# Bing-Jing/Ape-X

Measured on AMD Instinct MI355X. Metric: learner SGD steps/sec + actor frames/sec, Ape-X DQN Atari at 1/2/4/8 MI355X, higher is better.
Workload: dtype fp32

## Files before the change

### ape-x_amd/ops/csrc/f32_kernels.hip

```cpp
#include <algorithm>
#include <cstdio>
#include <cstdlib>
#include <type_traits>

#include "common.h"
#include "kernels.h"
#include "tree_dev.h"

namespace apex {
namespace {

typedef float f32x16 __attribute__((ext_vector_type(16)));
typedef float f32x4 __attribute__((ext_vector_type(4)));

__device__ __forceinline__ f32x4 ld4(const float* p) { return *reinterpret_cast<const f32x4*>(p); }
__device__ __forceinline__ f32x4 zero4() { return f32x4{0.f, 0.f, 0.f, 0.f}; }
__device__ __forceinline__ f32x4 u8x4(uint32_t w) {
  return f32x4{(float)(w & 0xFFu), (float)((w >> 8) & 0xFFu), (float)((w >> 16) & 0xFFu), (float)(w >> 24)};
}

constexpr int kPlane = 84 * 84;

typedef __amdgpu_buffer_rsrc_t Rsrc;
__device__ __forceinline__ Rsrc make_rsrc(const void* p, uint32_t nbytes) {
// ... 779 lines not shown
    return {(uint32_t)(((c.m0 + row) * 3136 + 4 * ch) * 4)};
  }
  static __device__ f32x4 load_a_row(const Args&, const Ctx& c, const RowA& r, int kb) {
    return bld4(c.in, r.off + (uint32_t)(kb * BK * 4));
  }
  static __device__ RowB row_b(const Args&, const Ctx& c, int nl, int ch) {
    return {(uint32_t)(((c.n0 + nl) * 3136 + 4 * ch) * 4)};
  }
  static __device__ f32x4 load_b_row(const Args&, const Ctx& c, const RowB& r, int kb) {
    return bld4(c.w, r.off + (uint32_t)(kb * BK * 4));
  }
};

constexpr int kPlaneDw = kPlane / 4;

struct W1Split {
  bfx8 hi[8], mid[8], lo[8];
};

__device__ __forceinline__ void split_w1(const float* wrow, W1Split& w) {
#pragma unroll
  for (int kb = 0; kb < 8; ++kb) {
    const f32x4 v0 = ld4(wrow + 32 * kb), v1 = ld4(wrow + 32 * kb + 8);
    const float x[8] = {v0[0], v0[1], v0[2], v0[3], v1[0], v1[1], v1[2], v1[3]};
    uint32_t h[4], m[4], l[4];
#pragma unroll
    for (int j = 0; j < 4; ++j) {
      const float a = x[2 * j], b = x[2 * j + 1];
      const float ah = trunc_bf16(a), bh = trunc_bf16(b);
      const float ar = a - ah, br = b - bh;
      const float am = trunc_bf16(ar), bm = trunc_bf16(br);
      h[j] = pack_bf16_hi(ah, bh);
      m[j] = pack_bf16_hi(am, bm);
      l[j] = pack_bf16_hi(ar - am, br - bm);
    }
    w.hi[kb] = __builtin_bit_cast(bfx8, make_uint4(h[0], h[1], h[2], h[3]));
    w.mid[kb] = __builtin_bit_cast(bfx8, make_uint4(m[0], m[1], m[2], m[3]));
    w.lo[kb] = __builtin_bit_cast(bfx8, make_uint4(l[0], l[1], l[2], l[3]));
  }
}

constexpr int kC1xGrid = 512;
constexpr int kC1xGridLearner = 384;
constexpr int kC1xDrawMax = 8;
constexpr int kC1xChunks = 4 * (kPlane / 16), kC1xPer = (kC1xChunks + 255) / 256;

__device__ __forceinline__ void c1x_load(const F32Set& set, int smp, uint4 (&v)[kC1xPer], const int* fid) {
  const int B = set.B, prob = smp / B, b = smp - prob * B, t = threadIdx.x;
  const F32Prob p = pick(set, prob);
  const uint8_t* fr = static_cast<const uint8_t*>(p.in);
  const FrameSrc f{fr, p.ids, p.idx};
  const uint4* s0 = reinterpret_cast<const uint4*>(fid ? fr + (size_t)fid[0] * kPlane : frame_plane(f, b, 0, kPlane));
  const uint4* s1 = reinterpret_cast<const uint4*>(fid ? fr + (size_t)fid[1] * kPlane : frame_plane(f, b, 1, kPlane));
  const uint4* s2 = reinterpret_cast<const uint4*>(fid ? fr + (size_t)fid[2] * kPlane : frame_plane(f, b, 2, kPlane));
  const uint4* s3 = reinterpret_cast<const uint4*>(fid ? fr + (size_t)fid[3] * kPlane : frame_plane(f, b, 3, kPlane));
#pragma unroll
  for (int k = 0; k < kC1xPer; ++k) {
    const int e = min(t + 256 * k, kC1xChunks - 1), c = e / 441;
    const uint4* sc = c == 0 ? s0 : (c == 1 ? s1 : (c == 2 ? s2 : s3));
    v[k] = sc[e - c * 441];
  }
}

__device__ __forceinline__ void c1x_store(const uint4 (&v)[kC1xPer], uint32_t* xs) {
  const int t = threadIdx.x;
#pragma unroll
  for (int k = 0; k < kC1xPer; ++k) {
    const int e = t + 256 * k;
    if (e < kC1xChunks) {
      const f32x4 a = u8x4(v[k].x), bq = u8x4(v[k].y), c = u8x4(v[k].z), d = u8x4(v[k].w);
      uint4* dst = reinterpret_cast<uint4*>(xs) + 2 * e;
      dst[0] = make_uint4(pack_bf16_hi(a[0], a[1]), pack_bf16_hi(a[2], a[3]), pack_bf16_hi(bq[0], bq[1]),
                          pack_bf16_hi(bq[2], bq[3]));
      dst[1] = make_uint4(pack_bf16_hi(c[0], c[1]), pack_bf16_hi(c[2], c[3]), pack_bf16_hi(d[0], d[1]),
                          pack_bf16_hi(d[2], d[3]));
    }
  }
}

__device__ __forceinline__ int opaque_i(int x) {
  asm volatile("" : "+v"(x));
  return x;
}
template <bool BITS>
__global__ __launch_bounds__(256, 2) void f32_conv1_fwd_x3_k(F32Set set, ConvSample cs) {
  __shared__ __attribute__((aligned(16))) uint32_t xs[2 * kPlaneDw * 4];
  __shared__ int fid[kC1xDrawMax][4];
  const int B = set.B, total = set.n * B;
  const int t = threadIdx.x, lane = t & 63, wave = t >> 6;
  const int i = lane & 15, q = lane >> 4, nh = wave >> 1;
  const bool draw = cs.out_idx != nullptr;
  const int G = draw ? cs.nhost : (int)gridDim.x;
  if (draw && (int)blockIdx.x >= G) {
    staged_scatter(cs.rows, blockIdx.x - G);
    return;
  }
  const __bf16* xb = reinterpret_cast<const __bf16*>(xs);
  W1Split w;
  int cur = -1;
  uint4 v[kC1xPer];
  const int per = (total + G - 1) / G;
  const int s0 = blockIdx.x * per, s1 = min(total, s0 + per);
  if (draw) {
    for (int k = wave; k < s1 - s0; k += 4) {
      const int smp = s0 + k, prob = smp / B, b = smp - prob * B;
      const int64_t len64 = cs.length[0];
      const int length = (int)(len64 < (int64_t)cs.t.size[0] ? len64 : (int64_t)cs.t.size[0]);
      const float pmin = cs.t.node_min[cs.t.levels - 1][0];
      float p;
      const int node = tree_sample_leaf(cs.t, b, B, length, cs.exclude_last, cs.seed, (uint64_t)cs.counter[0], lane,
                                        &p);
      const int se = staged_row_of(cs.rows, node, lane);
      const F32Prob pp = pick(set, prob);
      const int* ids = se < 0 ? pp.ids : (pp.ids == cs.rows.dst.s_ids ? cs.rows.st.s_ids : cs.rows.st.s2_ids);
      const int srow = se < 0 ? node : se;
      const bool crow = prob == 0 && cs.batch_fid != nullptr;
      uint32_t f = 0;
      if (lane < 4) {
        f = (uint32_t)ids[4 * srow + lane];
      } else if (crow && lane < 7) {
        const void* col = lane == 4 ? (const void*)(se < 0 ? cs.src_act : cs.rows.st.action)
                                    : (lane == 5 ? (const void*)(se < 0 ? cs.src_rew : cs.rows.st.reward)
                                                 : (const void*)(se < 0 ? cs.src_done : cs.rows.st.done));
        f = static_cast<const uint32_t*>(col)[srow];
      }
      if (lane < 4) fid[k][lane] = (int)f;
      if (prob == 0 && lane == 0) {
        cs.out_idx[b] = node;
        cs.out_w[b] = per_is_weight(p, pmin, 1.f, cs.beta[0]);
      }
      if (crow) {
        if (lane < 4) {
          cs.batch_fid[4 * b + lane] = (int)f;
        } else if (lane < 7) {
          void* dst = lane == 4 ? (void*)cs.batch_act : (lane == 5 ? (void*)cs.batch_rew : (void*)cs.batch_done);
          static_cast<uint32_t*>(dst)[b] = f;
        }
      }
    }
    __syncthreads();
  }
  if (s0 < s1) c1x_load(set, s0, v, draw ? fid[0] : nullptr);
  for (int smp = s0; smp < s1; ++smp) {
    const int prob = smp / B, b = smp - prob * B;
    const F32Prob p = pick(set, prob);
    if (prob != cur) {
      cur = prob;
      split_w1(p.w + (nh * 16 + i) * 256 + (q >> 1) * 16 + (q & 1) * 4, w);
    }
    __syncthreads();
    c1x_store(v, xs);
    __syncthreads();
    if (smp + 1 < s1) c1x_load(set, smp + 1, v, draw ? fid[smp + 1 - s0] : nullptr);
    float* out = p.out + (size_t)b * 400 * 32 + nh * 16 + 4 * q;
    uint16_t* bits =
        BITS && p.relu_bits ? reinterpret_cast<uint16_t*>(p.relu_bits + (size_t)b * 400) + nh : nullptr;
    float4 bias4;
    bias4.x = p.bias[nh * 16 + 4 * q];
    bias4.y = p.bias[nh * 16 + 4 * q + 1];
    bias4.z = p.bias[nh * 16 + 4 * q + 2];
    bias4.w = p.bias[nh * 16 + 4 * q + 3];
    auto frags = [&](int tile, bfx8 (&a)[8]) {
      const int m = tile * 16 + i, oy = m / 20, ox = m - oy * 20;
      const __bf16* a0 = xb + (4 * oy + 2 * (q >> 1)) * 84 + 4 * ox + 4 * (q & 1);
#pragma unroll
      for (int kb = 0; kb < 8; ++kb) {
        const uint2* ap = reinterpret_cast<const uint2*>(a0 + (kb >> 1) * kPlane + (kb & 1) * 4 * 84);
        const uint2 lo = ap[0], hi = ap[opaque_i(21)];
        a[kb] = __builtin_bit_cast(bfx8, make_uint4(lo.x, lo.y, hi.x, hi.y));
      }
    };
    auto tile_mfma = [&](int tile, const bfx8 (&a)[8], auto WB) {
      f32x4 ah = zero4(), am = zero4(), al = zero4();
#pragma unroll
      for (int kb = 0; kb < 8; ++kb) {
        ah = __builtin_amdgcn_mfma_f32_16x16x32_bf16(w.hi[kb], a[kb], ah, 0, 0, 0);
        am = __builtin_amdgcn_mfma_f32_16x16x32_bf16(w.mid[kb], a[kb], am, 0, 0, 0);
        al = __builtin_amdgcn_mfma_f32_16x16x32_bf16(w.lo[kb], a[kb], al, 0, 0, 0);
      }
      float4 y;
      y.x = fmaxf(ah[0] + (am[0] + al[0]) + bias4.x, 0.f);
      y.y = fmaxf(ah[1] + (am[1] + al[1]) + bias4.y, 0.f);
      y.z = fmaxf(ah[2] + (am[2] + al[2]) + bias4.z, 0.f);
      y.w = fmaxf(ah[3] + (am[3] + al[3]) + bias4.w, 0.f);
      *reinterpret_cast<float4*>(out + (size_t)(tile * 16 + i) * 32) = y;
      if constexpr (decltype(WB)::value) {
        const unsigned long long b0 = __ballot(y.x > 0.f), b1 = __ballot(y.y > 0.f), b2 = __ballot(y.z > 0.f),
                                 b3 = __ballot(y.w > 0.f);
        auto lo = [&](unsigned long long b) { return ((uint32_t)b >> i) & 0x00010001u; };
        auto hi = [&](unsigned long long b) { return ((uint32_t)(b >> 32) >> i) & 0x00010001u; };
        const uint32_t T = lo(b0) | lo(b1) << 1 | lo(b2) << 2 | lo(b3) << 3;
        const uint32_t U = hi(b0) | hi(b1) << 1 | hi(b2) << 2 | hi(b3) << 3;
        const uint32_t nb = (T & 0xFu) | ((T >> 12) & 0xF0u) | ((U & 0xFu) << 8) | ((U >> 4) & 0xF000u);
        bits[(tile * 16 + i) * 2] = (uint16_t)nb;
      }
    };
    auto tiles = [&](auto WB) {
      bfx8 fa[8], fb[8];
      const int t0 = wave & 1;
      frags(t0, fa);
      for (int pr = 0; pr < 6; ++pr) {
        const int tile = t0 + 4 * pr;
        frags(tile + 2, fb);
        tile_mfma(tile, fa, WB);
        frags(min(tile + 4, 24), fa);
        tile_mfma(tile + 2, fb, WB);
      }
      if (t0 == 0) tile_mfma(24, fa, WB);
    };
    if constexpr (BITS) {
      if (__builtin_amdgcn_readfirstlane(bits != nullptr)) tiles(std::true_type{});
      else tiles(std::false_type{});
    } else {
      tiles(std::false_type{});
    }
  }
}

struct BwdArgs {
  const void* x;
  const int* ids;
  const int* idx;
  const float* dy;
  const float* w;
  const float* mask;
  const uint32_t* mask_bits;
  const int* batch_fid;
  float* out;
  float* out2;
  int B;
  int kbps;
  int splits;
};

struct Fc1Dgrad {
  static constexpr int BM = 64, BN = 64, BK = 32, WM = 2;
  static constexpr bool A_KMAJ = true, B_KMAJ = false, SMEM = false;
  using Args = BwdArgs;
  using Smem = NoSmem;
  struct Ctx {
    int m0, n0, kb0, kb1;
    Rsrc dy, w;
  };
  static __host__ __device__ int tiles(int B) { return ((B + BM - 1) / BM) * 49; }
  static __device__ void decode(const Args& a, int block, Ctx& c, Smem&) {
    c.n0 = (block % 49) * BN;
    c.m0 = (block / 49) * BM;
    c.kb0 = 0;
    c.kb1 = 256 / BK;
    c.dy = make_rsrc(a.dy, (uint32_t)a.B * 256 * 4);
    c.w = make_rsrc(a.w, 256 * 3136 * 4);
  }
  using RowA = BufRow;
  using RowB = BufRow;
  static __device__ RowA row_a(const Args&, const Ctx& c, int row, int ch) {
    return {(uint32_t)((c.m0 + row) * 256 + 4 * ch) * 4};
  }
  static __device__ f32x4 load_a_row(const Args&, const Ctx& c, const RowA& r, int kb) {
    return bld4(c.dy, r.off + (uint32_t)(kb * BK * 4));
  }
  static __device__ RowB row_b(const Args&, const Ctx& c, int row, int ch) {
    return {(uint32_t)(row * 3136 + c.n0 + 4 * ch) * 4};
  }
  static __device__ f32x4 load_b_row(const Args&, const Ctx& c, const RowB& r, int kb) {
    return bld4(c.w, r.off + (uint32_t)(kb * BK * 3136 * 4));
  }
  static __device__ void store(const Args& a, const Ctx& c, int ml, int nl, float v) {
    const int b = c.m0 + ml;
    if (b >= a.B) return;
    const size_t o = (size_t)b * 3136 + c.n0 + nl;
    a.out[o] = a.mask[o] > 0.f ? v : 0.f;
  }
  static constexpr bool MASK_BITS = true;
  static __host__ __device__ bool use_bits(const Args& a) { return a.mask_bits != nullptr; }
  static __device__ uint32_t mask_word(const Args& a, const Ctx& c, int ml, int nl0) {
    return a.mask_bits[(size_t)min(c.m0 + ml, a.B - 1) * 98 + ((c.n0 + nl0) >> 5)];
  }
  static __device__ void store_keep(const Args& a, const Ctx& c, int ml, int nl, float v, bool keep) {
    const int b = c.m0 + ml;
    if (b < a.B) a.out[(size_t)b * 3136 + c.n0 + nl] = keep ? v : 0.f;
  }
};

struct Fc1Wgrad {
  static constexpr int BM = 64, BN = 64, BK = 32, WM = 2;
  static constexpr bool A_KMAJ = false, B_KMAJ = false, SMEM = false;
  using Args = BwdArgs;
  using Smem = NoSmem;
  struct Ctx {
// ... 362 lines not shown
  static __device__ RowB row_b(const Args&, const Ctx&, int n, int ch) { return {(uint32_t)(n * 64 + 4 * ch) * 4}; }
  static __device__ f32x4 load_b_row(const Args&, const Ctx& c, const RowB& r, int kb) {
    int ty, tx;
    tap_of(c, kb, ty, tx);
    const int ky = (c.cls >> 1) + 2 * ty, kx = (c.cls & 1) + 2 * tx;
    return bld4(c.w, r.off + (uint32_t)(((ky * 4 + kx) * 32 * 64 + (kb % KPT) * BK) * 4));
  }
  static __device__ void store(const Args& a, const Ctx& c, int ml, int n, float v) {
    const int b = c.b0 + ml;
    if (b >= a.B) return;
    const int iy = 2 * c.jy + (c.cls >> 1), ix = 2 * c.jx + (c.cls & 1);
    const size_t o = ((size_t)b * 400 + iy * 20 + ix) * 32 + n;
    a.out[o] = a.mask[o] > 0.f ? v : 0.f;
  }
  static constexpr bool MASK_BITS = true;
  static __host__ __device__ bool use_bits(const Args& a) { return a.mask_bits != nullptr; }
  static __device__ uint32_t mask_word(const Args& a, const Ctx& c, int ml, int) {
    const int iy = 2 * c.jy + (c.cls >> 1), ix = 2 * c.jx + (c.cls & 1);
    return a.mask_bits[(size_t)min(c.b0 + ml, a.B - 1) * 400 + iy * 20 + ix];
  }
  static __device__ void store_keep(const Args& a, const Ctx& c, int ml, int n, float v, bool keep) {
    const int b = c.b0 + ml;
    if (b >= a.B) return;
    const int iy = 2 * c.jy + (c.cls >> 1), ix = 2 * c.jx + (c.cls & 1);
    a.out[((size_t)b * 400 + iy * 20 + ix) * 32 + n] = keep ? v : 0.f;
  }
};
using Conv2DgradP = Conv2DgradPT<16>;
using Conv2DgradP32 = Conv2DgradPT<32>;

constexpr int kStageSplitDefault = 3 + 4 * 3 + 16 * (0 + 1);
constexpr int kBwdTileDefault = 1;

struct SplitPlan {
  int splits, kbps;
};

SplitPlan plan_splits(int kbt, int ntiles, int target_blocks) {
  int s = std::max(1, target_blocks / ntiles);
  int kbps = std::max(1, (kbt + s - 1) / s);
  s = (kbt + kbps - 1) / kbps;
  return {s, kbps};
}

SplitPlan wgrad_plan(int layer, int B, int target) {
  switch (layer) {
    case 1: {
      const int S = target == 1 ? 1 : kConv1WgradS;
      return {(B + S - 1) / S, S};
    }
    case 2: return plan_splits(ConvWgrad<2>::kblocks(B), 512 / 64, target > 0 ? target : 256);
    case 3: return plan_splits(ConvWgrad<3>::kblocks(B), 576 / 64, target > 0 ? target : 252);
    default: throw std::invalid_argument("f32 wgrad layer");
  }
}

int g_stage_split = -1;
int stage_split_mask() {
  if (g_stage_split < 0) {
    const char* e = std::getenv("APEX_F32_STAGE_SPLIT");
    g_stage_split = e ? std::atoi(e) : kStageSplitDefault;
  }
  return g_stage_split;
}

constexpr int kPrefetchDefault = 0;
int g_prefetch = -1;
int prefetch_mask() {
  if (g_prefetch < 0) {
    const char* e = std::getenv("APEX_F32_PREFETCH");
    g_prefetch = e ? std::atoi(e) : kPrefetchDefault;
  }
  return g_prefetch;
}
constexpr int kBatchResolveDefault = 1;
int g_batch_resolve = -1;
int batch_resolve_mask() {
  if (g_batch_resolve < 0) {
    const char* e = std::getenv("APEX_F32_BATCH_RESOLVE");
    g_batch_resolve = e ? std::atoi(e) & 3 : kBatchResolveDefault;
  }
  return g_batch_resolve;
}
int prefetch_depth(int cls) { return std::min(3, 1 + ((prefetch_mask() >> (2 * cls)) & 3)); }

template <class P, int D, bool XB>
void launch1_d(const typename P::Args& a, int blocks, hipStream_t s, int form) {
  switch (form) {
    case 1: gemm_k<P, 1, D, XB><<<blocks, 256, 0, s>>>(a); break;
    case 2: gemm_k<P, 2, D, XB><<<blocks, 256, 0, s>>>(a); break;
    case 3: gemm_k<P, 3, D, XB><<<blocks, 256, 0, s>>>(a); break;
    default: gemm_k<P, 0, D, XB><<<blocks, 256, 0, s>>>(a);
  }
}
template <class P, bool XB>
void launch1_x(const typename P::Args& a, int blocks, hipStream_t s, bool small) {
  const int m = stage_split_mask();
  const int form = small && ((m >> 4) & 3) ? ((m >> 4) & 3) - 1 : m & 3;
  switch (prefetch_depth(small ? 2 : 0)) {
    case 2: launch1_d<P, 2, XB>(a, blocks, s, form); break;
    case 3: launch1_d<P, 3, XB>(a, blocks, s, form); break;
    default: launch1_d<P, 1, XB>(a, blocks, s, form);
  }
}
template <class P>
void launch1(const typename P::Args& a, int blocks, hipStream_t s, bool small = false, bool bits = false) {
  if (blocks <= 0) return;
  if constexpr (HasReluBits<P>::value) {
    if (bits) launch1_x<P, true>(a, blocks, s, small);
    else launch1_x<P, false>(a, blocks, s, small);
  } else {
    launch1_x<P, false>(a, blocks, s, small);
  }
  LAUNCH_CHECK();
}

template <class P1, class P2, int D, bool XB>
void launch2_d(const typename P1::Args& a1, const typename P2::Args& a2, int n1, int nb, const TreeRide& r,
               hipStream_t s) {
  switch ((stage_split_mask() >> 2) & 3) {
    case 1: gemm2_k<P1, P2, 1, D, XB><<<nb, 256, 0, s>>>(a1, a2, n1, r); break;
    case 2: gemm2_k<P1, P2, 2, D, XB><<<nb, 256, 0, s>>>(a1, a2, n1, r); break;
    case 3: gemm2_k<P1, P2, 3, D, XB><<<nb, 256, 0, s>>>(a1, a2, n1, r); break;
    default: gemm2_k<P1, P2, 0, D, XB><<<nb, 256, 0, s>>>(a1, a2, n1, r);
  }
}
template <class P1, class P2, bool XB>
void launch2_x(const typename P1::Args& a1, const typename P2::Args& a2, int n1, int nb, const TreeRide& r,
               hipStream_t s) {
  switch (prefetch_depth(1)) {
    case 2: launch2_d<P1, P2, 2, XB>(a1, a2, n1, nb, r, s); break;
    case 3: launch2_d<P1, P2, 3, XB>(a1, a2, n1, nb, r, s); break;
    default: launch2_d<P1, P2, 1, XB>(a1, a2, n1, nb, r, s);
  }
}

template <class P1, class P2>
void launch2(const typename P1::Args& a1, int n1, const typename P2::Args& a2, int n2, hipStream_t s,
             const TreeRide* ride = nullptr) {
  if (n1 + n2 <= 0) return;
  TreeRide r{};
  if (ride && ride->stage) {
    r = *ride;
    r.nhost = n1 + n2;
  }
  const int nb = n1 + n2 + tree_ride_blocks(r);
  if (P2::use_bits(a2)) launch2_x<P1, P2, true>(a1, a2, n1, nb, r, s);
  else launch2_x<P1, P2, false>(a1, a2, n1, nb, r, s);
  LAUNCH_CHECK();
}

void check_set(const F32Set& set) {
  if (set.n < 1 || set.n > kMaxProbs) throw std::invalid_argument("f32: 1..3 problems");
  if (set.B <= 0) throw std::invalid_argument("f32: B must be positive");
  if ((int64_t)(set.B + 128) * 400 * 32 * 4 >= (int64_t)1 << 31)
    throw std::invalid_argument("f32: batch too large for 32-bit operand offsets");
}

template <class P>
void fwd_launch(const F32Set& set, hipStream_t s) {
  launch1<P>(set, set.n * P::tiles(set.B), s, set.n * set.B < 1024, set.p[0].relu_bits != nullptr);
}

}

void f32_set_stage_split(int mask) { g_stage_split = mask; }
int f32_stage_split() { return stage_split_mask(); }
void f32_set_prefetch(int mask) { g_prefetch = mask; }
int f32_prefetch() { return prefetch_mask(); }
void f32_set_batch_resolve(int mask) { g_batch_resolve = mask < 0 ? -1 : mask & 3; }
int f32_batch_resolve() { return batch_resolve_mask(); }

static bool learner_sized(const F32Set& set) { return set.n * set.B >= 1024; }

static int default_tile(int layer) {
  static int t2 = -1, t3 = -1;
  if (t2 < 0) {
    t2 = t3 = 0;
    if (const char* e = std::getenv("APEX_F32_TILES")) std::sscanf(e, "%d%*c%d", &t2, &t3);
  }
  return layer == 2 ? t2 : t3;
}

void f32_conv_fwd_multi(int layer, const F32Set& set, hipStream_t s, int c1_grid, int tile, const ConvSample* draw) {
  check_set(set);
  if (draw && draw->out_idx && layer != 1) throw std::invalid_argument("f32_conv_fwd_multi: the draw folds into conv1");
  if (tile == 0 && (layer == 2 || layer == 3)) tile = default_tile(layer);
  switch (layer) {
    case 1: {
      if (c1_grid <= 0) c1_grid = learner_sized(set) ? kC1xGridLearner : (set.n * set.B + 1) / 2;
      const int G = std::min(set.n * set.B, c1_grid > 0 ? c1_grid : kC1xGrid);
      ConvSample c{};
      if (draw && draw->out_idx) {
        c = *draw;
        c.nhost = G;
        if ((set.n * set.B + G - 1) / G > kC1xDrawMax)
          throw std::invalid_argument("f32 conv1 draw: <= 8 samples per workgroup");
        if (!c.length || !c.beta || !c.counter || !c.out_w || set.p[0].idx != c.out_idx)
          throw std::invalid_argument("f32 conv1 draw: fill level, beta, counter, weights, and problem 0 reading idx");
        if (c.batch_fid && (!c.batch_act || !c.batch_rew || !c.batch_done || !c.src_act || !c.src_rew || !c.src_done))
          throw std::invalid_argument("f32 conv1 draw: the compact rows need all four outputs and the table columns");
        for (int k = 0; k < set.n; ++k)
          if (!set.p[k].ids || (c.rows.E > 0 && set.p[k].ids != c.rows.dst.s_ids && set.p[k].ids != c.rows.dst.s2_ids))
            throw std::invalid_argument("f32 conv1 draw: every problem reads the replay's frame-id tables");
      }
      const int nb = G + (c.out_idx ? (c.rows.E + 255) / 256 : 0);
      if (set.p[0].relu_bits) f32_conv1_fwd_x3_k<true><<<nb, 256, 0, s>>>(set, c);
      else f32_conv1_fwd_x3_k<false><<<nb, 256, 0, s>>>(set, c);
      LAUNCH_CHECK();
      break;
    }
    case 2:
      if (learner_sized(set) && tile == 1) fwd_launch<Conv2FwdT<64, 64, 32, 2>>(set, s);
      else if (learner_sized(set) && tile == 2) fwd_launch<Conv2FwdT<128, 64, 32, 4>>(set, s);
      else if (learner_sized(set)) fwd_launch<Conv2FwdT<128, 64, 32, 2>>(set, s);
      else fwd_launch<Conv2FwdT<128, 32, 32, 4>>(set, s);
      break;
    case 3:
      if (learner_sized(set) && tile == 2) fwd_launch<Conv3FwdT<128, 64, 32, 2>>(set, s);
      else if (learner_sized(set) && tile == 3) fwd_launch<Conv3FwdT<128, 32, 32, 4>>(set, s);
      else if (learner_sized(set)) fwd_launch<Conv3FwdT<64, 64, 32, 2>>(set, s);
      else fwd_launch<Conv3FwdT<128, 64, 32, 2>>(set, s);
      break;
    default: throw std::invalid_argument("f32_conv_fwd_multi: layer must be 1, 2 or 3");
  }
}

int f32_fc1_splits() { return kFcSplits; }

int f32_fc1_fwd_multi(const F32Set& set, hipStream_t s) {
  check_set(set);
  fwd_launch<Fc1FwdT<64, 64, 32, 2>>(set, s);
  return kFcSplits;
}

constexpr int kFc1WgSlices = 1;

int f32_fc1_wgrad_splits() { return kFc1WgSlices; }

size_t f32_fc1_wgrad_workspace_floats() { return (size_t)kFc1WgSlices * 256 * 3136; }

static void check_bwd_batch(int B) {
  if ((int64_t)B * 400 * 32 * 4 + (int64_t)64 * 400 * 32 * 4 >= (int64_t)1 << 31)
    throw std::invalid_argument("f32 backward: batch too large for 32-bit operand offsets");
}

void f32_fc1_bwd_split(const float* dz, const float* a3, const float* wfc1p, float* dy3, float* ws, int B,
                       hipStream_t s, const TreeRide* ride, const uint32_t* mask_bits) {
  if (B <= 0) return;
  check_bwd_batch(B);
  BwdArgs d{};
  d.dy = dz;
  d.w = wfc1p;
  d.mask = a3;
  d.mask_bits = mask_bits;
  d.out = dy3;
  d.B = B;
  BwdArgs w{};
  w.x = a3;
  w.dy = dz;
  w.out = ws;
  w.B = B;
  const int nkb = (B + Fc1Wgrad::BK - 1) / Fc1Wgrad::BK;
  w.splits = std::min(kFc1WgSlices, nkb);
  w.kbps = (nkb + w.splits - 1) / w.splits;
  w.splits = (nkb + w.kbps - 1) / w.kbps;
  launch2<Fc1Wgrad, Fc1Dgrad>(w, Fc1Wgrad::tiles(B) * w.splits, d, Fc1Dgrad::tiles(B), s, ride);
}

int f32_fc1_wgrad_slices(int B) {
  const int nkb = (B + Fc1Wgrad::BK - 1) / Fc1Wgrad::BK;
  const int g = std::min(kFc1WgSlices, nkb), kbps = (nkb + g - 1) / g;
  return (nkb + kbps - 1) / kbps;
}

int f32_wgrad_splits(int layer, int B, int target) { return wgrad_plan(layer, B, target).splits; }

int f32_wgrad_kbps(int layer, int B, int target) { return wgrad_plan(layer, B, target).kbps; }

size_t f32_wgrad_workspace_floats(int layer, int B, int target) {
  const SplitPlan p = wgrad_plan(layer, B, target);
  const size_t per = layer == 1 ? 32 * 256 : (layer == 2 ? 64 * 512 : 64 * 576);
  const size_t cout = layer == 1 ? 32 : 64;
  return (size_t)p.splits * (per + cout);
}

void f32_conv_bwd(int layer, const void* x, const int* ids, const int* idx, const float* dy, const float* w,
                  const float* mask, float* dx, float* ws, int B, hipStream_t s, int target, int tile,
                  const TreeRide* ride, const uint32_t* mask_bits, const int* batch_fid) {
  if (B <= 0) return;
  check_bwd_batch(B);
// ... 95 lines not shown
```

### ape-x_amd/ops/csrc/hip_bindings.cpp

```cpp
#include <pybind11/pybind11.h>
#include <pybind11/stl.h>

#include <array>
#include <optional>
#include <vector>

#include "common.h"
#include "kernels.h"

namespace py = pybind11;
using namespace apex;

namespace {

template <typename T>
T* P(uint64_t v) {
  return reinterpret_cast<T*>(static_cast<uintptr_t>(v));
}
hipStream_t S(uint64_t v) { return reinterpret_cast<hipStream_t>(static_cast<uintptr_t>(v)); }

struct TreeHandle {
  TreeDesc d{};
};

// ... 431 lines not shown
        !a.delta || !a.lw || !(a.dz_bf || a.dz) || !a.part || !a.step)
      throw std::invalid_argument("dqn_heads_bwd: missing pointer");
    dqn_heads_bwd(a, S(s));
  });
  m.def("conv_wgrad", [](int layer, uint64_t x, uint64_t ids, uint64_t idx, uint64_t dy, uint64_t dy_mask, int B,
                         uint64_t ws, uint64_t grad, uint64_t bgrad, uint64_t s) {
    conv_wgrad(layer, P<const void>(x), P<const int>(ids), P<const int>(idx), P<const uint16_t>(dy),
               P<const uint16_t>(dy_mask), B, P<float>(ws), P<float>(grad), P<float>(bgrad), S(s));
  });
  m.def("pack_conv_wt", [](uint64_t src, uint64_t dst, int N, int C, int KH, int KW, uint64_t s) {
    pack_conv_wt(P<const float>(src), P<uint16_t>(dst), N, C, KH, KW, S(s));
  });
  auto f32set = [](const std::vector<std::vector<uint64_t>>& probs, int B) {
    if (probs.empty() || probs.size() > (size_t)kMaxProbs) throw std::invalid_argument("1..3 problems");
    F32Set set{};
    for (size_t i = 0; i < probs.size(); ++i) {
      const auto& t = probs[i];
      if (t.size() != 7 && t.size() != 8) throw std::invalid_argument("f32 problem: 7 or 8 fields");
      set.p[i] = F32Prob{P<const void>(t[0]), P<const int>(t[1]), P<const int>(t[2]), P<const float>(t[3]),
                         P<const float>(t[4]), P<const float>(t[5]), P<float>(t[6]),
                         t.size() == 8 ? P<uint32_t>(t[7]) : nullptr};
      if (set.p[i].relu_bits && i != 0) throw std::invalid_argument("f32 problem: sign bits are problem 0's");
    }
    set.n = (int)probs.size();
    set.B = B;
    return set;
  };
  m.def("f32_conv_fwd_multi", [f32set](int layer, const std::vector<std::vector<uint64_t>>& probs, int B,
                                       uint64_t s, int c1_grid, int tile, py::object draw) {
    f32_conv_fwd_multi(layer, f32set(probs, B), S(s), c1_grid, tile,
                       draw.is_none() ? nullptr : draw.cast<const ConvSample*>());
  }, py::arg("layer"), py::arg("probs"), py::arg("B"), py::arg("s"), py::arg("c1_grid") = 0, py::arg("tile") = 0,
     py::arg("draw") = py::none());
  py::class_<ConvSample>(m, "ConvSample");
  m.def("make_conv_sample", [](const TreeHandle& t, uint64_t length_ptr, uint64_t beta_ptr, uint64_t seed,
                               uint64_t counter, uint64_t out_idx, uint64_t out_w, int exclude_last,
                               py::object rows_stage, py::object rows_dst, uint64_t rows_slot, uint64_t rows_prio,
                               int rows_E, uint64_t batch_fid, uint64_t batch_act, uint64_t batch_rew,
                               uint64_t batch_done, py::object batch_src) {
    if (!length_ptr || !beta_ptr || !counter || !out_idx || !out_w)
      throw std::invalid_argument("make_conv_sample: fill level, beta, counter, idx and weight pointers");
    ConvSample c{};
    c.t = t.d;
    c.length = P<const int64_t>(length_ptr);
    c.beta = P<const float>(beta_ptr);
    c.counter = P<const int64_t>(counter);
    c.seed = seed;
    c.out_idx = P<int>(out_idx);
    c.out_w = P<float>(out_w);
    c.exclude_last = exclude_last;
    if (rows_E > 0) {
      if (!rows_slot || !rows_prio) throw std::invalid_argument("make_conv_sample: staged slots / priorities");
      c.rows = StagedRows{trans_table(rows_stage.cast<py::dict>()), trans_table(rows_dst.cast<py::dict>()),
                          P<const int>(rows_slot), P<const float>(rows_prio), rows_E};
    }
    if (batch_fid) {
      if (!batch_act || !batch_rew || !batch_done || batch_src.is_none())
        throw std::invalid_argument("make_conv_sample: compact rows need fid, act, rew, done and the table");
      const TransTable src = trans_table(batch_src.cast<py::dict>());
      c.batch_fid = P<int>(batch_fid);
      c.batch_act = P<int>(batch_act);
      c.batch_rew = P<float>(batch_rew);
      c.batch_done = P<float>(batch_done);
      c.src_act = src.action;
      c.src_rew = src.reward;
      c.src_done = src.done;
    }
    return c;
  }, py::arg("t"), py::arg("length_ptr"), py::arg("beta_ptr"), py::arg("seed"), py::arg("counter"),
     py::arg("out_idx"), py::arg("out_w"), py::arg("exclude_last"), py::arg("rows_stage") = py::none(),
     py::arg("rows_dst") = py::none(), py::arg("rows_slot") = 0, py::arg("rows_prio") = 0, py::arg("rows_E") = 0,
     py::arg("batch_fid") = 0, py::arg("batch_act") = 0, py::arg("batch_rew") = 0, py::arg("batch_done") = 0,
     py::arg("batch_src") = py::none());
  m.def("f32_fc1_fwd_multi", [f32set](const std::vector<std::vector<uint64_t>>& probs, int B, uint64_t s) {
    return f32_fc1_fwd_multi(f32set(probs, B), S(s));
  });
  m.def("f32_fc1_splits", &f32_fc1_splits);
  m.def("f32_set_stage_split", &f32_set_stage_split);
  m.def("f32_stage_split", &f32_stage_split);
  m.def("f32_set_prefetch", &f32_set_prefetch);
  m.def("f32_prefetch", &f32_prefetch);
  m.def("f32_set_batch_resolve", &f32_set_batch_resolve);
  m.def("f32_batch_resolve", &f32_batch_resolve);
  m.def("f32_fc1_bwd_split", [](uint64_t dz, uint64_t a3, uint64_t wfc1p, uint64_t dy3, uint64_t ws, int B,
                                uint64_t s, py::object ride, uint64_t mask_bits) {
    f32_fc1_bwd_split(P<const float>(dz), P<const float>(a3), P<const float>(wfc1p), P<float>(dy3), P<float>(ws), B,
                      S(s), ride_of(ride), P<const uint32_t>(mask_bits));
  }, py::arg("dz"), py::arg("a3"), py::arg("wfc1p"), py::arg("dy3"), py::arg("ws"), py::arg("B"), py::arg("s"),
     py::arg("ride") = py::none(), py::arg("mask_bits") = 0);
  m.def("f32_fc1_wgrad_splits", &f32_fc1_wgrad_splits);
  m.def("f32_fc1_wgrad_slices", &f32_fc1_wgrad_slices);
  m.def("f32_fc1_wgrad_workspace_floats", &f32_fc1_wgrad_workspace_floats);
  m.def("f32_fc1_finalize_job", [](int half, int G, uint64_t ws, uint64_t grad) {
    return f32_fc1_finalize_job(half, G, P<const float>(ws), P<float>(grad));
  });
  m.def("f32_wgrad_splits", &f32_wgrad_splits, py::arg("layer"), py::arg("B"), py::arg("target") = 0);
  m.def("f32_wgrad_kbps", &f32_wgrad_kbps, py::arg("layer"), py::arg("B"), py::arg("target") = 0);
  m.def("f32_wgrad_workspace_floats", &f32_wgrad_workspace_floats, py::arg("layer"), py::arg("B"),
        py::arg("target") = 0);
  m.def("f32_conv_bwd", [](int layer, uint64_t x, uint64_t ids, uint64_t idx, uint64_t dy, uint64_t w, uint64_t mask,
                           uint64_t dx, uint64_t ws, int B, uint64_t s, int target, int tile, py::object ride,
                           uint64_t mask_bits, uint64_t batch_fid) {
    f32_conv_bwd(layer, P<const void>(x), P<const int>(ids), P<const int>(idx), P<const float>(dy), P<const float>(w),
                 P<const float>(mask), P<float>(dx), P<float>(ws), B, S(s), target, tile, ride_of(ride),
                 P<const uint32_t>(mask_bits), P<const int>(batch_fid));
  }, py::arg("layer"), py::arg("x"), py::arg("ids"), py::arg("idx"), py::arg("dy"), py::arg("w"), py::arg("mask"),
     py::arg("dx"), py::arg("ws"), py::arg("B"), py::arg("s"), py::arg("target") = 0, py::arg("tile") = 0,
     py::arg("ride") = py::none(), py::arg("mask_bits") = 0, py::arg("batch_fid") = 0);
  m.def("f32_conv_finalize_job", [](int layer, int B, uint64_t ws, uint64_t grad, uint64_t bgrad, int target) {
    return f32_conv_finalize_job(layer, B, P<const float>(ws), P<float>(grad), P<float>(bgrad), target);
  }, py::arg("layer"), py::arg("B"), py::arg("ws"), py::arg("grad"), py::arg("bgrad"), py::arg("target") = 0);
  m.def("norm_only_job", [](uint64_t g, int n) { return norm_only_job(P<const float>(g), n); });

  m.def("create_dedicated_stream", [](int device) {
    auto hip_ok = [](hipError_t e) {
      if (e != hipSuccess) throw std::runtime_error(std::string("create_dedicated_stream: ") + hipGetErrorString(e));
    };
    int cus = 0;
    hip_ok(hipDeviceGetAttribute(&cus, hipDeviceAttributeMultiprocessorCount, device));
    std::vector<uint32_t> mask((cus + 31) / 32, 0xFFFFFFFFu);
    if (cus % 32) mask.back() = (1u << (cus % 32)) - 1u;
    int prev = 0;
    hip_ok(hipGetDevice(&prev));
    hip_ok(hipSetDevice(device));
    hipStream_t st = nullptr;
    hip_ok(hipExtStreamCreateWithCUMask(&st, (uint32_t)mask.size(), mask.data()));
    hip_ok(hipSetDevice(prev));
    return (uint64_t)reinterpret_cast<uintptr_t>(st);
  });
  m.def("spin_us", [](int us, uint64_t s) { spin_us(us, S(s)); });

  m.def("event_create", [](bool light) {
    hipEvent_t e;
    HIP_CHECK(hipEventCreateWithFlags(&e, hipEventDisableTiming | (light ? hipEventDisableSystemFence : 0u)));
    return reinterpret_cast<uint64_t>(e);
  });
  m.def("event_record", [](uint64_t e, uint64_t s) {
    HIP_CHECK(hipEventRecord(reinterpret_cast<hipEvent_t>(e), S(s)));
  });
  m.def("stream_wait_event", [](uint64_t s, uint64_t e) {
    HIP_CHECK(hipStreamWaitEvent(S(s), reinterpret_cast<hipEvent_t>(e), 0));
  });
  m.def("event_destroy", [](uint64_t e) { HIP_CHECK(hipEventDestroy(reinterpret_cast<hipEvent_t>(e))); });
  m.def("copy_f32", [](uint64_t dst, uint64_t src, int64_t n, uint64_t s) {
    copy_f32(P<float>(dst), P<const float>(src), n, S(s));
  });

  py::class_<AQLNet>(m, "AQLNet");
  m.def("make_aql_net", [](py::dict ints, py::dict ptrs) {
    AQLNet n{};
    auto gi = [&](const char* k) { return ints[k].cast<int>(); };
    n.obs = gi("obs"); n.adim = gi("adim"); n.cont = gi("cont"); n.T = gi("T"); n.na = gi("na");
    n.uniform = gi("uniform"); n.propose = gi("propose"); n.noisy = gi("noisy");
    auto gp = [&](const char* k) -> const float* {
      return ptrs.contains(k) ? reinterpret_cast<const float*>(ptrs[k].cast<uint64_t>()) : nullptr;
    };
    n.qf_w1 = gp("qf_w1"); n.qf_b1 = gp("qf_b1"); n.qf_w2 = gp("qf_w2"); n.qf_b2 = gp("qf_b2");
    n.ao_w1 = gp("ao_w1"); n.ao_b1 = gp("ao_b1"); n.ao_w2 = gp("ao_w2"); n.ao_b2 = gp("ao_b2");
    n.a1_wmu = gp("a1_wmu"); n.a1_wsig = gp("a1_wsig"); n.a1_weps = gp("a1_weps");
    n.a1_bmu = gp("a1_bmu"); n.a1_bsig = gp("a1_bsig"); n.a1_beps = gp("a1_beps");
    n.a2_wmu = gp("a2_wmu"); n.a2_wsig = gp("a2_wsig"); n.a2_weps = gp("a2_weps");
    n.a2_bmu = gp("a2_bmu"); n.a2_bsig = gp("a2_bsig"); n.a2_beps = gp("a2_beps");
    n.f_w = gp("f_w"); n.f_b = gp("f_b");
    n.df_w1 = gp("df_w1"); n.df_b1 = gp("df_b1"); n.df_w2 = gp("df_w2"); n.df_b2 = gp("df_b2");
    if (!n.qf_w1 || !n.ao_w1 || !n.a1_wmu || !n.a2_wmu) throw std::invalid_argument("make_aql_net: missing weights");
    if (n.cont && (!n.ao_w2 || n.adim < 1)) throw std::invalid_argument("make_aql_net: continuous encoder");
// ... 486 lines not shown
```

### ape-x_amd/ops/csrc/kernels.h

```cpp
#pragma once

#include <hip/hip_runtime.h>

#include <cstdint>

namespace apex {

constexpr int kTreeFanout = 64;
constexpr int kTreeLog2Fanout = 6;
constexpr int kMaxTreeLevels = 8;

struct TreeDesc {
  float* leaf_sum;
  float* leaf_min;
  double* node_sum[kMaxTreeLevels];
  float* node_min[kMaxTreeLevels];
  int size[kMaxTreeLevels + 1];
  int levels;
};
struct ShardGlob {
  const float* slots;
  int world, rank;
};
struct PrioMix {
// ... 253 lines not shown
               const float* b_adv2, const float* w_val2, const float* b_val2, float* hout, float* q, int B, int A,
               hipStream_t s);
int fc1_splits();
int fc1_splits_for(int total_rows);
int fc1_fwd(const uint16_t* a, const uint16_t* w, float* part, int B, hipStream_t s);
struct FcProb {
  const uint16_t* a;
  const uint16_t* w;
  float* part;
};
struct FcSet {
  FcProb p[kMaxProbs];
  int n, B;
};
int fc1_fwd_multi(const FcSet& set, hipStream_t s);
int fc1_bwd_slices();
size_t fc1_bwd_workspace_floats();
void fc1_bwd(const uint16_t* dz, const uint16_t* a3, const uint16_t* wt, uint16_t* dy3, float* part, int B,
             hipStream_t s);
struct HeadsProb {
  const float* z;
  const float *b_adv1, *b_val1, *w_adv2, *b_adv2, *w_val2, *b_val2;
  float* hout;
  float* q;
};
struct ActSel {
  const float* eps;
  const int64_t* counter;
  int* actions;
  uint64_t seed;
};
struct HeadsSet {
  HeadsProb p[kMaxProbs];
  int n, B, A, nsplit;
  int xcd_map;
  ActSel act;
};
void heads_fwd_multi(const HeadsSet& set, hipStream_t s);
void heads_bwd(const float* dq, const float* h, const float* w_adv2, const float* w_val2, float* dA, float* dz,
               uint16_t* dz_bf, int B, int A, hipStream_t s);
void pack_conv_w(const float* src, uint16_t* dst, int N, int C, int KH, int KW, hipStream_t s);
void pack_fc1(const float* adv, const float* val, uint16_t* dst, int P, int C, hipStream_t s);
void unpack_fc1_grad(const float* gp, float* g_adv, float* g_val, int P, int C, hipStream_t s);
void relu_mask_bf16(const uint16_t* g, const uint16_t* a, uint16_t* out, int64_t n, hipStream_t s);
void u8_to_bf16_nhwc(const uint8_t* in, uint16_t* out, int B, int HW, hipStream_t s);

void conv_dgrad(int layer, const uint16_t* dy, const uint16_t* dy_mask, const uint16_t* wt, uint16_t* dx,
                const uint16_t* dx_mask, int B, hipStream_t s);
size_t wgrad_workspace_floats(int layer);
void conv_wgrad(int layer, const void* x, const int* ids, const int* idx, const uint16_t* dy, const uint16_t* dy_mask,
                int B, float* workspace, float* grad, float* bias_grad, hipStream_t s);
void pack_conv_wt(const float* src, uint16_t* dst, int N, int C, int KH, int KW, hipStream_t s);


void conv1_fwd_multi(const ConvSet& set, hipStream_t s);
void conv1_fwd(const uint8_t* frames, const int* ids, const int* idx, const uint16_t* w, const float* bias,
               uint16_t* out, int B, hipStream_t s);

struct F32Prob {
  const void* in;
  const int* ids;
  const int* idx;
  const float* w;
  const float* w2;
  const float* bias;
  float* out;
  uint32_t* relu_bits;
};
struct F32Set {
  F32Prob p[kMaxProbs];
  int n, B;
};
struct ConvSample {
  TreeDesc t;
  const int64_t* length;
  const float* beta;
  const int64_t* counter;
  uint64_t seed;
  int* out_idx;
  float* out_w;
  int exclude_last;
  StagedRows rows;
  int nhost;
  int* batch_fid;
  int* batch_act;
  float* batch_rew;
  float* batch_done;
  const int* src_act;
  const float* src_rew;
  const float* src_done;
};
void f32_conv_fwd_multi(int layer, const F32Set& set, hipStream_t s, int c1_grid = 0, int tile = 0,
                        const ConvSample* draw = nullptr);
int f32_fc1_splits();
void f32_set_stage_split(int mask);
int f32_stage_split();
void f32_set_prefetch(int mask);
int f32_prefetch();
void f32_set_batch_resolve(int mask);
int f32_batch_resolve();
int f32_fc1_fwd_multi(const F32Set& set, hipStream_t s);
int f32_wgrad_splits(int layer, int B, int target = 0);
int f32_wgrad_kbps(int layer, int B, int target = 0);
size_t f32_wgrad_workspace_floats(int layer, int B, int target = 0);
int f32_fc1_wgrad_splits();
int f32_fc1_wgrad_slices(int B);
size_t f32_fc1_wgrad_workspace_floats();
void f32_fc1_bwd_split(const float* dz, const float* a3, const float* wfc1p, float* dy3, float* ws, int B,
                       hipStream_t s, const TreeRide* ride = nullptr, const uint32_t* mask_bits = nullptr);
void f32_conv_bwd(int layer, const void* x, const int* ids, const int* idx, const float* dy, const float* w,
                  const float* mask, float* dx, float* ws, int B, hipStream_t s, int target = 0, int tile = 0,
                  const TreeRide* ride = nullptr,
                  const uint32_t* mask_bits = nullptr,
                  const int* batch_fid = nullptr);
FinalizeJob f32_conv_finalize_job(int layer, int B, const float* ws, float* grad, float* bias_grad, int target = 0);
FinalizeJob norm_only_job(const float* g, int n);

struct AQLNet {
  int obs, adim, cont, T, na, uniform, propose, noisy;
  const float *qf_w1, *qf_b1, *qf_w2, *qf_b2;
  const float *ao_w1, *ao_b1, *ao_w2, *ao_b2;
  const float *a1_wmu, *a1_wsig, *a1_weps, *a1_bmu, *a1_bsig, *a1_beps;
  const float *a2_wmu, *a2_wsig, *a2_weps, *a2_bmu, *a2_bsig, *a2_beps;
  const float *f_w, *f_b;
  const float *df_w1, *df_b1, *df_w2, *df_b2;
};
size_t aql_workspace_floats();
void aql_noisy_eff(const AQLNet& net, float* ws, hipStream_t s);
void aql_candidate_q(const AQLNet& net, float* ws, const float* state, const float* a_mu, int B, float* q,
                     hipStream_t s);
void aql_propose(const AQLNet& net, const float* state, int B, const float* low, const float* high, const float* var,
                 uint64_t seed, const int64_t* counter, float* a_mu, float* mu_out, hipStream_t s,
                 float* eff_ws = nullptr);
void aql_select(const float* q, const float* a_mu, int B, int T, int adim, const float* eps, uint64_t seed,
                const int64_t* counter, int* act_idx, float* env_act, hipStream_t s);

namespace aqlv {
constexpr int GQ = 0, H = 8, GH = 72, X = 136, GX = 264, AOH = 392, GAOH = 520, A = 648, QFH = 656, GQFH = 720,
              S = 784, EMB = 848, HID = 976, GHID = 1104, GMU = 1232, STRIDE = 1296;
}
constexpr int kAqlMaxJobs = 32;
struct AqlLearn {
  AQLNet on, tg;
  const float *eff_on, *eff_tg;
  const float *st, *st2, *rew, *done, *amu;
  const int* act;
  const int* idx;
  const float* w;
  int B;
  float gamma_n, ent_lam;
  const float* var;
  float *q_s, *q_s2, *qt_s2;
  float* vec;
  float *delta, *lw, *lossp;
  long long* dbg;
  int act_mode;
  int act_blocks;
  int fused_sample, exclude_last;
  TreeDesc tree;
  const int64_t* filled;
  const float* beta;
  const int64_t* ctr;
  uint64_t seed;
  int* idx_out;
  float* w_out;
  int bwd_tree;
  int bwd_levels;
  BatchWrite bw;
  int tile_groups;
  int fwd_halves;
  const int* gate;
  int gate_j;
};
void aql_learn_fwd(const AqlLearn& L, hipStream_t s);
void aql_act_q(const AqlLearn& L, hipStream_t s);
void aql_learn_bwd(const AqlLearn& L, hipStream_t s);
struct AqlGradJob {
  int64_t off;
  int rows, cols;
  int goff, xoff;
  const float* eps;
  int group;
  int zero;
// ... 333 lines not shown
```

Before: 2728.

## Pair conv1 problems 1 and 2 in shared workgroups that reuse one staged input

When problems 1 and 2 of the conv1 forward read the same frames (same input, ids and idx, no relu bits), a pair of workgroups processes each sample once for both problems. Each wave takes one problem's half of the channels and walks all tiles, instead of loading the frames separately per problem. The pair/single workgroup split is set by a configurable share. The change also adds a kernarg prefetch touch and restricts relu-bit stores to a single lane group. It adds another template variant and a host heuristic for sizing the grid.

After: 2755 (median of 6 runs). Within noise of the previous version (+1.0%).

```diff
diff --git a/ape-x_amd/ops/csrc/f32_kernels.hip b/ape-x_amd/ops/csrc/f32_kernels.hip
--- a/ape-x_amd/ops/csrc/f32_kernels.hip
+++ b/ape-x_amd/ops/csrc/f32_kernels.hip
@@ -885,13 +885,23 @@
   asm volatile("" : "+v"(x));
   return x;
 }
-template <bool BITS>
+__device__ __forceinline__ void c1x_touch_args() {
+  typedef const uint32_t __attribute__((address_space(4))) * KArg;
+  KArg ka = (KArg)__builtin_amdgcn_kernarg_segment_ptr();
+  constexpr int kBytes = (int)((sizeof(F32Set) + 7) / 8 * 8 + sizeof(ConvSample));
+  uint32_t any = 0;
+#pragma unroll
+  for (int l = 0; l <= (kBytes - 4) / 64; ++l) any |= ka[16 * l];
+  asm volatile("" ::"s"(any));
+}
+template <bool BITS, bool PAIR>
 __global__ __launch_bounds__(256, 2) void f32_conv1_fwd_x3_k(F32Set set, ConvSample cs) {
   __shared__ __attribute__((aligned(16))) uint32_t xs[2 * kPlaneDw * 4];
   __shared__ int fid[kC1xDrawMax][4];
   const int B = set.B, total = set.n * B;
   const int t = threadIdx.x, lane = t & 63, wave = t >> 6;
-  const int i = lane & 15, q = lane >> 4, nh = wave >> 1;
+  const int i = lane & 15, q = lane >> 4;
+  c1x_touch_args();
   const bool draw = cs.out_idx != nullptr;
   const int G = draw ? cs.nhost : (int)gridDim.x;
   if (draw && (int)blockIdx.x >= G) {
@@ -902,8 +912,22 @@
   W1Split w;
   int cur = -1;
   uint4 v[kC1xPer];
-  const int per = (total + G - 1) / G;
-  const int s0 = blockIdx.x * per, s1 = min(total, s0 + per);
+  int s0, s1;
+  bool pw = false;
+  if constexpr (PAIR) {
+    const int g0 = cs.pair_g0;
+    pw = (int)blockIdx.x >= g0;
+    const int nwg = pw ? G - g0 : g0, r = pw ? (int)blockIdx.x - g0 : (int)blockIdx.x;
+    const int per = (B + nwg - 1) / nwg;
+    s0 = min(B, r * per) + (pw ? B : 0);
+    s1 = min(B + (pw ? B : 0), s0 + per);
+  } else {
+    const int per = (total + G - 1) / G;
+    s0 = blockIdx.x * per;
+    s1 = min(total, s0 + per);
+  }
+  const int wv = PAIR ? __builtin_amdgcn_readfirstlane(wave) : wave;
+  const int nh = PAIR && pw ? wv & 1 : wave >> 1;
   if (draw) {
     for (int k = wave; k < s1 - s0; k += 4) {
       const int smp = s0 + k, prob = smp / B, b = smp - prob * B;
@@ -945,7 +969,8 @@
   }
   if (s0 < s1) c1x_load(set, s0, v, draw ? fid[0] : nullptr);
   for (int smp = s0; smp < s1; ++smp) {
-    const int prob = smp / B, b = smp - prob * B;
+    const int sprob = smp / B, b = smp - sprob * B;
+    const int prob = PAIR && pw ? 1 + (wv >> 1) : sprob;
     const F32Prob p = pick(set, prob);
     if (prob != cur) {
       cur = prob;
@@ -995,19 +1020,19 @@
         const uint32_t T = lo(b0) | lo(b1) << 1 | lo(b2) << 2 | lo(b3) << 3;
         const uint32_t U = hi(b0) | hi(b1) << 1 | hi(b2) << 2 | hi(b3) << 3;
         const uint32_t nb = (T & 0xFu) | ((T >> 12) & 0xF0u) | ((U & 0xFu) << 8) | ((U >> 4) & 0xF000u);
-        bits[(tile * 16 + i) * 2] = (uint16_t)nb;
+        if (q == 0) bits[(tile * 16 + i) * 2] = (uint16_t)nb;
       }
     };
     auto tiles = [&](auto WB) {
       bfx8 fa[8], fb[8];
-      const int t0 = wave & 1;
+      const int t0 = PAIR && pw ? 0 : wave & 1, st = PAIR && pw ? 1 : 2, np = PAIR && pw ? 12 : 6;
       frags(t0, fa);
-      for (int pr = 0; pr < 6; ++pr) {
-        const int tile = t0 + 4 * pr;
-        frags(tile + 2, fb);
+      for (int pr = 0; pr < np; ++pr) {
+        const int tile = t0 + 2 * st * pr;
+        frags(tile + st, fb);
         tile_mfma(tile, fa, WB);
-        frags(min(tile + 4, 24), fa);
-        tile_mfma(tile + 2, fb, WB);
+        frags(min(tile + 2 * st, 24), fa);
+        tile_mfma(tile + st, fb, WB);
       }
       if (t0 == 0) tile_mfma(24, fa, WB);
     };
@@ -1536,6 +1561,20 @@
   }
   return g_batch_resolve;
 }
+constexpr int kC1PairDefault = 1, kC1xSplitDefault = 128;
+int g_c1_pair = -1, g_c1_split = -1;
+static int env_knob(const char* name, int dflt) {
+  const char* e = std::getenv(name);
+  return e ? std::atoi(e) : dflt;
+}
+int c1_pair_on() {
+  if (g_c1_pair < 0) g_c1_pair = env_knob("APEX_F32_C1_PAIR", kC1PairDefault) != 0;
+  return g_c1_pair;
+}
+int c1_split_share() {
+  if (g_c1_split < 0) g_c1_split = std::max(0, env_knob("APEX_F32_C1_SPLIT", 0));
+  return g_c1_split;
+}
 int prefetch_depth(int cls) { return std::min(3, 1 + ((prefetch_mask() >> (2 * cls)) & 3)); }
 
 template <class P, int D, bool XB>
@@ -1624,6 +1663,12 @@
 int f32_prefetch() { return prefetch_mask(); }
 void f32_set_batch_resolve(int mask) { g_batch_resolve = mask < 0 ? -1 : mask & 3; }
 int f32_batch_resolve() { return batch_resolve_mask(); }
+void f32_set_c1_chain(int pair, int split) {
+  if (pair >= 0) g_c1_pair = pair != 0;
+  if (split >= 0) g_c1_split = split;
+}
+int f32_c1_pair() { return c1_pair_on(); }
+int f32_c1_split() { return c1_split_share(); }
 
 static bool learner_sized(const F32Set& set) { return set.n * set.B >= 1024; }
 
@@ -1645,10 +1690,16 @@
       if (c1_grid <= 0) c1_grid = learner_sized(set) ? kC1xGridLearner : (set.n * set.B + 1) / 2;
       const int G = std::min(set.n * set.B, c1_grid > 0 ? c1_grid : kC1xGrid);
       ConvSample c{};
+      const F32Prob &p1 = set.p[1], &p2 = set.p[2];
+      const bool pair = c1_pair_on() && set.n == 3 && G >= 2 && p1.in == p2.in && p1.ids == p2.ids &&
+                        p1.idx == p2.idx && !p1.relu_bits && !p2.relu_bits;
+      const int share = c1_split_share() > 0 ? c1_split_share() : kC1xSplitDefault;
+      const int g0 = pair ? std::max(1, std::min(G - 1, (int)(((int64_t)G * share + 192) / 384))) : 0;
+      const int run = pair ? std::max((set.B + g0 - 1) / g0, (set.B + G - g0 - 1) / (G - g0)) : (set.n * set.B + G - 1) / G;
       if (draw && draw->out_idx) {
         c = *draw;
         c.nhost = G;
-        if ((set.n * set.B + G - 1) / G > kC1xDrawMax)
+        if (run > kC1xDrawMax)
           throw std::invalid_argument("f32 conv1 draw: <= 8 samples per workgroup");
         if (!c.length || !c.beta || !c.counter || !c.out_w || set.p[0].idx != c.out_idx)
           throw std::invalid_argument("f32 conv1 draw: fill level, beta, counter, weights, and problem 0 reading idx");
@@ -1659,8 +1710,11 @@
             throw std::invalid_argument("f32 conv1 draw: every problem reads the replay's frame-id tables");
       }
       const int nb = G + (c.out_idx ? (c.rows.E + 255) / 256 : 0);
-      if (set.p[0].relu_bits) f32_conv1_fwd_x3_k<true><<<nb, 256, 0, s>>>(set, c);
-      else f32_conv1_fwd_x3_k<false><<<nb, 256, 0, s>>>(set, c);
+      c.pair_g0 = g0;
+      if (pair && set.p[0].relu_bits) f32_conv1_fwd_x3_k<true, true><<<nb, 256, 0, s>>>(set, c);
+      else if (pair) f32_conv1_fwd_x3_k<false, true><<<nb, 256, 0, s>>>(set, c);
+      else if (set.p[0].relu_bits) f32_conv1_fwd_x3_k<true, false><<<nb, 256, 0, s>>>(set, c);
+      else f32_conv1_fwd_x3_k<false, false><<<nb, 256, 0, s>>>(set, c);
       LAUNCH_CHECK();
       break;
     }
diff --git a/ape-x_amd/ops/csrc/hip_bindings.cpp b/ape-x_amd/ops/csrc/hip_bindings.cpp
--- a/ape-x_amd/ops/csrc/hip_bindings.cpp
+++ b/ape-x_amd/ops/csrc/hip_bindings.cpp
@@ -537,6 +537,9 @@
   m.def("f32_prefetch", &f32_prefetch);
   m.def("f32_set_batch_resolve", &f32_set_batch_resolve);
   m.def("f32_batch_resolve", &f32_batch_resolve);
+  m.def("f32_set_c1_chain", &f32_set_c1_chain, py::arg("pair") = -1, py::arg("split") = -1);
+  m.def("f32_c1_pair", &f32_c1_pair);
+  m.def("f32_c1_split", &f32_c1_split);
   m.def("f32_fc1_bwd_split", [](uint64_t dz, uint64_t a3, uint64_t wfc1p, uint64_t dy3, uint64_t ws, int B,
                                 uint64_t s, py::object ride, uint64_t mask_bits) {
     f32_fc1_bwd_split(P<const float>(dz), P<const float>(a3), P<const float>(wfc1p), P<float>(dy3), P<float>(ws), B,
diff --git a/ape-x_amd/ops/csrc/kernels.h b/ape-x_amd/ops/csrc/kernels.h
--- a/ape-x_amd/ops/csrc/kernels.h
+++ b/ape-x_amd/ops/csrc/kernels.h
@@ -359,6 +359,7 @@
   int exclude_last;
   StagedRows rows;
   int nhost;
+  int pair_g0;
   int* batch_fid;
   int* batch_act;
   float* batch_rew;
@@ -376,6 +377,9 @@
 int f32_prefetch();
 void f32_set_batch_resolve(int mask);
 int f32_batch_resolve();
+void f32_set_c1_chain(int pair, int split);
+int f32_c1_pair();
+int f32_c1_split();
 int f32_fc1_fwd_multi(const F32Set& set, hipStream_t s);
 int f32_wgrad_splits(int layer, int B, int target = 0);
 int f32_wgrad_kbps(int layer, int B, int target = 0);
```
